# xuekt98/BBDM

Hardware: AMD Instinct MI355X
Metric: denoise-UNet sampling steps/sec (one step = p_sample of the whole local batch: UNet forward + Brownian-Bridge update) at 256x256 pixel-space BBDM (higher is better)
Workload: dtype f32 (tile GEMMs: fp32 operands as two fp16 planes under a provable power-of-two scale, 3 fp16-MFMA terms, fp32 accumulate -- measured against fp64 MORE accurate than the six-term bf16x3 split and than the f32 MFMA; 1x1 layers (skip / qkv / proj_out) and the long-sequence attention: the same pair; sh; 1 GPU; pixel-space BBDM 256x256, batch 16, 1000-step schedule (BASELINE.json configs[1]); batch_per_gpu=16, image_size=256, schedule_steps=1000, parallelism=dp1 (independent image-pair shards)

## Files before the change

bbdm_amd/csrc/common.h:

```cpp
#pragma once
#include <hip/hip_runtime.h>
#include <stdint.h>
#include <stdio.h>
#include "../../include/bbdm_hip.h"

typedef float f32x4 __attribute__((ext_vector_type(4)));
typedef float f32x16 __attribute__((ext_vector_type(16)));

#define BBDM_WAVE 64

void bbdm_set_error(const char* fmt, ...);

enum BbdmOption { BBDM_OPT_WGRAD1X1_BF3 = 0, BBDM_OPT_WINO_IDX64, BBDM_OPT_BF3P_KERNEL, BBDM_OPT_ATTN_BF3, BBDM_OPT_ATTN_PIPE, BBDM_OPT_BF3P_PAD_ROWS, BBDM_OPT_COUNT };
int bbdm_option(int id);

#define BBDM_REQUIRE(cond, ...)            \
    do {                                   \
        if (!(cond)) {                     \
            bbdm_set_error(__VA_ARGS__);   \
            return BBDM_E_BADARG;          \
        }                                  \
    } while (0)

#define BBDM_CHECK_LAUNCH(what)                                                        \
    do {                                                                               \
        hipError_t e__ = hipGetLastError();                                            \
        if (e__ != hipSuccess) {                                                       \
            bbdm_set_error("%s: launch failed: %s", what, hipGetErrorString(e__));     \
            return BBDM_E_LAUNCH;                                                      \
        }                                                                              \
    } while (0)

constexpr int BBDM_MAX_DEVICES = 64;
static inline int bbdm_device_slot() {
    int d = 0;
    if (hipGetDevice(&d) != hipSuccess || d < 0 || d >= BBDM_MAX_DEVICES) d = 0;
    return d;
}
template <auto Kernel>
static inline int bbdm_ensure_lds(size_t bytes, const char* what) {
    static size_t set_dev[BBDM_MAX_DEVICES] = {};
    size_t& set = set_dev[bbdm_device_slot()];
    if (bytes <= set) return BBDM_OK;
    if (hipFuncSetAttribute(reinterpret_cast<const void*>(Kernel), hipFuncAttributeMaxDynamicSharedMemorySize, (int)bytes) != hipSuccess) {
        bbdm_set_error("%s: hipFuncSetAttribute(%zu B LDS) failed", what, bytes);
        return BBDM_E_LAUNCH;
    }
    set = bytes;
    return BBDM_OK;
}

int bbdm_gemm_tn_impl(const float* A, int lda, size_t a_stride, const float* B, int ldb, size_t b_stride, float* C, float* bias_part,
                      int batch, long long K, int M, int N, void* stream);

namespace {
__global__ void bbdm_zero8_kernel(unsigned long long* __restrict__ p, size_t n) {
    for (size_t i = blockIdx.x * (size_t)blockDim.x + threadIdx.x; i < n; i += (size_t)gridDim.x * blockDim.x) p[i] = 0ull;
}
}
static inline void bbdm_zero_async(void* p, size_t bytes, hipStream_t st) {
    const size_t n = bytes / 8;
    if (!n) return;
    size_t blocks = (n + 255) / 256;
    if (blocks > 2048) blocks = 2048;
    hipLaunchKernelGGL(bbdm_zero8_kernel, dim3((unsigned)blocks), dim3(256), 0, st, (unsigned long long*)p, n);
}
// ... 73 lines not shown
```

bbdm_amd/csrc/runtime.hip:

```cpp
#include <stdarg.h>
#include <string.h>
#include "common.h"

static thread_local char g_err[512] = "";

void bbdm_set_error(const char* fmt, ...) {
    va_list ap;
    va_start(ap, fmt);
    vsnprintf(g_err, sizeof(g_err), fmt, ap);
    va_end(ap);
}

extern "C" int bbdm_version(void) { return 33; }

namespace {
struct Option { const char* name; int value; };
Option g_options[BBDM_OPT_COUNT] = {
    {"wgrad1x1_bf3", 1},
    {"wino_idx64", 0},
    {"bf3p_kernel", 6},
    {"attn_bf3", 1},
    {"attn_pipe", 2},
    {"bf3p_pad_rows", 1},
};
int option_index(const char* name) {
    if (!name) return -1;
    for (int i = 0; i < BBDM_OPT_COUNT; ++i)
        if (strcmp(name, g_options[i].name) == 0) return i;
    return -1;
}
}
int bbdm_option(int id) { return g_options[id].value; }
extern "C" int bbdm_set_option(const char* name, int value) {
    const int i = option_index(name);
    BBDM_REQUIRE(i >= 0, "bbdm_set_option: unknown option '%s'", name ? name : "(null)");
    g_options[i].value = value;
    return BBDM_OK;
}
extern "C" int bbdm_get_option(const char* name, int* value) {
    const int i = option_index(name);
    BBDM_REQUIRE(i >= 0 && value, "bbdm_get_option: unknown option '%s' / null result", name ? name : "(null)");
    *value = g_options[i].value;
    return BBDM_OK;
}
extern "C" const char* bbdm_last_error(void) { return g_err; }

namespace {
int device_cus() {
    static int cus_dev[BBDM_MAX_DEVICES] = {};
    int& cus = cus_dev[bbdm_device_slot()];
    if (!cus) {
        int dev = 0;
        hipDeviceProp_t prop;
        cus = (hipGetDevice(&dev) == hipSuccess && hipGetDeviceProperties(&prop, dev) == hipSuccess && prop.multiProcessorCount > 0)
                  ? prop.multiProcessorCount : 256;
    }
    return cus;
}
}

extern "C" int bbdm_device_cus(void) { return device_cus(); }
```

bbdm_amd/csrc/winograd.hip:

```cpp
#include "winograd_math.h"
#include "dispatch.h"
#include <stdlib.h>
#include "bf3_split.h"
#include "h2_split.h"
#include "stats_acc.h"

namespace {

constexpr int KC = 16;

template <int MO, bool PRE, bool UP>
__global__ void __launch_bounds__(256) winograd_input_kernel(const float* __restrict__ x, int ldx, float* __restrict__ V,
                                                             const float* __restrict__ sc, const float* __restrict__ bi,
                                                             int pre_ld, int pre_silu, int N, int H, int W, int C,
                                                             size_t plane) {
    constexpr int AL = MO + 2;
    const int C4 = C >> 2;
    const int TH = H / MO, TW = W / MO;
    const long long total = (long long)N * TH * TW * C4;
    for (long long u = blockIdx.x * 256ll + threadIdx.x; u < total; u += (long long)gridDim.x * 256) {
        const int c = (int)(u % C4) * 4;
        const long long tile = u / C4;
        const int tw = (int)(tile % TW);
        const long long r = tile / TW;
// ... 208 lines not shown
            }
            bt_transform<MO>(d, col);
#pragma unroll
            for (int i = 0; i < AL; ++i) t[i][j] = col[i];
            __builtin_amdgcn_sched_barrier(0);
        }
        float* o = V + (size_t)tile * C + c;
#pragma unroll
        for (int i = 0; i < AL; ++i) {
            float2 row[AL];
            bt_transform<MO>(t[i], row);
#pragma unroll
            for (int j = 0; j < AL; ++j) { *reinterpret_cast<float2*>(o) = row[j]; o += plane; }
            __builtin_amdgcn_sched_barrier(0);
        }
    }
}


template <int AL, int NPL = 3>
__device__ __forceinline__ void store_transposed(const unsigned (&pl)[AL][NPL], unsigned char* scratch, int lane, unsigned char* dst_xi0,
                                                 size_t plane_t, int chunk, int tile0, int tchunks) {
    typedef short v4s __attribute__((ext_vector_type(4)));
    constexpr int HALF = AL / 2, COMBOS = NPL * HALF, PITCH = 256 + 64;
    static_assert(COMBOS * PITCH <= AL * 64 * 8, "transposition scratch exceeds the wave's LDS region");
    const int grp = lane >> 4, i16 = lane & 15;
    const int c = chunk * KC + i16;
    unsigned char* dst = dst_xi0 + (((size_t)(c >> 5) * tchunks + (tile0 >> 4)) * NPL) * 1024 + ((tile0 >> 3) & 1) * 512 + (c & 31) * 16;
#pragma unroll
    for (int round = 0; round < 2; ++round) {
        __builtin_amdgcn_wave_barrier();
#pragma unroll
        for (int q = 0; q < HALF; ++q)
#pragma unroll
            for (int p = 0; p < NPL; ++p)
                *reinterpret_cast<unsigned*>(scratch + (q * NPL + p) * PITCH + lane * 4) = pl[round * HALF + q][p];
        __builtin_amdgcn_wave_barrier();
#pragma unroll
        for (int it = 0; it < (COMBOS + 3) / 4; ++it) {
            const int combo = it * 4 + grp;
            const int cc = combo < COMBOS ? combo : COMBOS - 1;
            const unsigned char* a = scratch + cc * PITCH + (i16 >> 2) * 32 + (i16 & 3) * 8;
            const v4s lo = __builtin_amdgcn_ds_read_tr16_b64_v4i16((__attribute__((address_space(3))) v4s*)(a));
            const v4s hi = __builtin_amdgcn_ds_read_tr16_b64_v4i16((__attribute__((address_space(3))) v4s*)(a + 4 * 32));
            typedef short v8s __attribute__((ext_vector_type(8)));
            const v8s both = {lo[0], lo[1], lo[2], lo[3], hi[0], hi[1], hi[2], hi[3]};
            const int q = cc / NPL, p = cc - NPL * q;
            if (combo < COMBOS)
                *reinterpret_cast<uint4*>(dst + (size_t)(round * HALF + q) * plane_t + p * 1024) = __builtin_bit_cast(uint4, both);
        }
    }
}

struct GnFold {
    const unsigned long long* stats;
    const float* gamma;
    const float* beta;
    const float* film;
    int film_ld, C, G, cpg;
    double cnt;
    float eps;
};
template <int MO, bool PRE, bool UP, bool TR, bool IDX64, bool GNC = false, bool F32 = false, int ST = MO, int NPL = 3>
__global__ void __launch_bounds__((MO + 2) * 64) winograd_input_split2_kernel(const float* __restrict__ x, int ldx,
                                                                              unsigned char* __restrict__ Vp,
                                                                              const float* __restrict__ sc, const float* __restrict__ bi,
                                                                              int pre_ld, int pre_silu, int N, int H, int W, int nchunks,
                                                                              unsigned T, int TG, size_t plane,
                                                                              unsigned char* __restrict__ Vt, size_t plane_t,
                                                                              int tchunks, const FastDiv dTW, const FastDiv dTH,
                                                                              const FastDiv dCH, const GnFold gn,
                                                                              const float* __restrict__ hbound, int vt_h2 = 0) {
    static_assert(NPL == 3 || (NPL == 2 && !F32), "the fp16-pair planes have no fp32 form");
    constexpr int AL = MO + 2;
    __shared__ float2 lds[AL * AL * 64];
    const unsigned L = blockIdx.x, q = L >> 3;
    const unsigned qc = fastdiv(q, dCH);
    const int chunk = (int)(q - qc * (unsigned)nchunks), tg = (int)(qc * 8 + (L & 7));
    if (tg >= TG) return;
    const int lane = threadIdx.x & 63, wave = threadIdx.x >> 6;
    const int TH = (int)dTH.d, TW = (int)dTW.d;
    constexpr int TPG = F32 ? 4 : 8, CPW = F32 ? 16 : 8;
    const int tl = lane / CPW, cp = lane % CPW;
    const unsigned tile = (unsigned)tg * TPG + tl;
    const int c = chunk * (2 * CPW) + cp * 2;
    {
        const int jj = wave;
        float2 d[AL], col[AL];
        if (tile < T) {
            const unsigned r = fastdiv(tile, dTW), n = fastdiv(r, dTH);
            const int tw = (int)(tile - r * (unsigned)TW), th = (int)(r - n * (unsigned)TH);
            float2 s2 = make_float2(1.f, 1.f), b2 = make_float2(0.f, 0.f);
            if (PRE && GNC) {
                const unsigned long long* cell = gn.stats + (((size_t)n * gn.G + c / gn.cpg) * 2) * SA_W;
                const double s = sa_load(cell), ss = sa_load(cell + SA_W);
                const double mean = s / gn.cnt;
                double var = ss / gn.cnt - mean * mean;
                var = var > 0.0 ? var : 0.0;
                const float rstd = (float)(1.0 / sqrt(var + (double)gn.eps));
                const float fmean = (float)mean;
                const float2 ga = *reinterpret_cast<const float2*>(gn.gamma + c), be = *reinterpret_cast<const float2*>(gn.beta + c);
                float sc0 = rstd * ga.x, sc1 = rstd * ga.y;
                float bi0 = be.x - fmean * sc0, bi1 = be.y - fmean * sc1;
                if (gn.film) {
                    const float2 fs = *reinterpret_cast<const float2*>(gn.film + (size_t)n * gn.film_ld + c);
                    const float2 fb = *reinterpret_cast<const float2*>(gn.film + (size_t)n * gn.film_ld + gn.C + c);
                    sc0 = sc0 * (1.f + fs.x); sc1 = sc1 * (1.f + fs.y);
                    bi0 = bi0 * (1.f + fs.x) + fb.x; bi1 = bi1 * (1.f + fs.y) + fb.y;
                }
                s2 = make_float2(sc0, sc1);
                b2 = make_float2(bi0, bi1);
            } else if (PRE) {
                s2 = *reinterpret_cast<const float2*>(sc + (size_t)n * pre_ld + c);
                b2 = *reinterpret_cast<const float2*>(bi + (size_t)n * pre_ld + c);
            }
            const int Hs = UP ? H >> 1 : H, Ws = UP ? W >> 1 : W;
            const int w = ST * tw - 1 + jj;
            const int wc = min(max(w, 0), W - 1);
            const int wsrc = UP ? wc >> 1 : wc;
            const float wmask = (w >= 0 && w < W) ? 1.f : 0.f;
            const int h0 = ST * th - 1;
            if (IDX64) {
#pragma unroll
                for (int i = 0; i < AL; ++i) {
                    const int hc = min(max(h0 + i, 0), H - 1);
                    const int hs = UP ? hc >> 1 : hc;
                    d[i] = *reinterpret_cast<const float2*>(x + ((size_t)(n * Hs + hs) * Ws + wsrc) * ldx + c);
                }
            } else {
                const unsigned rowstride = (unsigned)Ws * (unsigned)ldx;
                const unsigned e0 = (n * (unsigned)Hs * (unsigned)Ws + (unsigned)wsrc) * (unsigned)ldx + (unsigned)c;
// ... 206 lines not shown
#pragma unroll
#if BBDM_NT_MLOAD
            for (int i = 0; i < AL; ++i) v[i] = load_nt(reinterpret_cast<const float2*>(m + (size_t)(i * AL + j) * plane));
#else
            for (int i = 0; i < AL; ++i) v[i] = *reinterpret_cast<const float2*>(m + (size_t)(i * AL + j) * plane);
#endif
            at_transform<MO>(v, sj);
#pragma unroll
            for (int a = 0; a < MO; ++a) s[a][j] = sj[a];
        }
        const float2 b2 = bias ? *reinterpret_cast<const float2*>(bias + c) : make_float2(0.f, 0.f);
        double psum = 0.0, psq = 0.0;
#pragma unroll
        for (int a = 0; a < MO; ++a) {
            float2 o[MO];
            at_transform<MO>(s[a], o);
            const int oh = MO * th + a;
            const int ohc = min(oh, H - 1);
            float2 rv[MO];
            if (RES) {
#pragma unroll
                for (int b = 0; b < MO; ++b) {
                    const int owc = min(MO * tw + b, W - 1);
                    const float* rp = res_per_image == 1 ? res + (size_t)n * ldr + c
                                      : res_per_image == 2 ? res + ((size_t)(n * (H >> 1) + (ohc >> 1)) * (W >> 1) + (owc >> 1)) * ldr + c
                                                           : res + ((size_t)(n * H + ohc) * W + owc) * ldr + c;
                    rv[b] = *reinterpret_cast<const float2*>(rp);
                }
            }
#pragma unroll
            for (int b = 0; b < MO; ++b) {
                const int ow = MO * tw + b;
                if (oh < H && ow < W) {
                    float2 val = o[b] + b2;
                    if (RES) val = val + rv[b];
                    const size_t pix = ph ? (size_t)(n * 2 * H + 2 * oh + (pq >> 1)) * (2 * W) + 2 * ow + (pq & 1)
                                          : (size_t)(n * H + oh) * W + ow;
                    *reinterpret_cast<float2*>(y + pix * ldy + c) = val;
                    if (stats) {
                        psum += (double)val.x + (double)val.y;
                        psq += (double)val.x * val.x + (double)val.y * val.y;
                    }
                }
            }
        }
        if (stats) stat_add(lsum, st, n - n0, n, c, psum, psq);
    }
    if (stats) {
        __syncthreads();
        stat_flush(lsum, st, n0, N);
    }
}

template <int MO, bool RES, int TPW, int AL = MO + 2>
__global__ void __launch_bounds__(AL * 64) winograd_output_lds_kernel(const float* __restrict__ M, size_t plane, int ldm, int splits,
                                                                   const float* __restrict__ bias,
                                                                   const float* __restrict__ res, int ldr, int res_per_image,
                                                                   float* __restrict__ y, int ldy, int N, int H, int W, int Cout,
                                                                   int cblocks, long long T, const StatArgs st, int ph, int tpw) {
    constexpr int NT = AL * 64, NBUF = TPW > 1 ? 2 : 1;
    constexpr int GL = 33;
    constexpr int TAB = MO * 2 * 2 * GL * 2;
    constexpr int XF = NBUF * MO * AL * 64;
    constexpr bool DYN = (size_t)XF * sizeof(float2) > 65536;
    __shared__ float2 lds_static[DYN ? 1 : (XF > TAB ? XF : TAB)];
    extern __shared__ __attribute__((aligned(16))) float2 lds_dynamic[];
    float2* const lds = DYN ? lds_dynamic : lds_static;
    const int lane = threadIdx.x & 63, wave = threadIdx.x >> 6;
    const int cb = (int)(blockIdx.x % (unsigned)cblocks);
    const long long tile0 = (long long)(blockIdx.x / (unsigned)cblocks) * tpw;
    const int TH = wino_tdim(H, MO), TW = wino_tdim(W, MO);
    const int n0 = (int)(tile0 / ((long long)TH * TW));
    const int cm = cb * 128 + 2 * lane;
    const int pq = ph ? cm / Cout : 0, c = cm - pq * Cout;
    const bool stats = st.s[0] != nullptr || st.s[1] != nullptr;
    double acc_s[2] = {0.0, 0.0}, acc_q[2] = {0.0, 0.0};
    const float2 b2 = bias ? *reinterpret_cast<const float2*>(bias + c) : make_float2(0.f, 0.f);
    for (int k = 0; k < tpw; ++k) {
        const long long tile = tile0 + k;
        if (tile >= T) break;
        float2* buf = lds + (k & (NBUF - 1)) * (MO * AL * 64);
        {
            const int j = wave;
            const float* m = M + (size_t)tile * ldm + cm + (size_t)j * plane;
            float2 v[AL], sj[MO];
#pragma unroll
            for (int i = 0; i < AL; ++i) v[i] = load_nt(reinterpret_cast<const float2*>(m + (size_t)(i * AL) * plane));
            for (int z = 1; z < splits; ++z)
#pragma unroll
                for (int i = 0; i < AL; ++i)
                    v[i] = v[i] + load_nt(reinterpret_cast<const float2*>(m + ((size_t)z * (AL * AL) + i * AL) * plane));
            if constexpr (MO == 7) at_transform7(v, sj); else at_transform<MO>(v, sj);
#pragma unroll
            for (int a = 0; a < MO; ++a) buf[(a * AL + j) * 64 + lane] = sj[a];
        }
        __syncthreads();
        if (wave < MO) {
            const int a = wave;
            const int tw = (int)(tile % TW);
            const long long r = tile / TW;
            const int th = (int)(r % TH), n = (int)(r / TH);
            float2 t[AL], o[MO];
#pragma unroll
            for (int j = 0; j < AL; ++j) t[j] = buf[(a * AL + j) * 64 + lane];
            const int oh = MO == 7 ? MO * th + a - (pq >> 1) : MO * th + a;
            if (oh < H && (MO != 7 || oh >= 0)) {
                float2 rv[MO];
                if (RES) {
#pragma unroll
                    for (int b = 0; b < MO; ++b) {
                        const int owc = min(MO * tw + b, W - 1);
                        const float* rp = res_per_image == 1 ? res + (size_t)n * ldr + c
                                          : res_per_image == 2 ? res + ((size_t)(n * (H >> 1) + (oh >> 1)) * (W >> 1) + (owc >> 1)) * ldr + c
                                                               : res + ((size_t)(n * H + oh) * W + owc) * ldr + c;
                        rv[b] = *reinterpret_cast<const float2*>(rp);
                    }
                }
                if constexpr (MO == 7) at_transform7(t, o); else at_transform<MO>(t, o);
                double psum = 0.0, psq = 0.0;
#pragma unroll
                for (int b = 0; b < MO; ++b) {
                    const int ow = MO == 7 ? MO * tw + b - (pq & 1) : MO * tw + b;
                    if (ow < W && (MO != 7 || ow >= 0)) {
                        float2 val = o[b] + b2;
                        if (RES) val = val + rv[b];
                        const size_t pix = ph ? (size_t)(n * 2 * H + 2 * oh + (pq >> 1)) * (2 * W) + 2 * ow + (pq & 1)
                                              : (size_t)(n * H + oh) * W + ow;
                        *reinterpret_cast<float2*>(y + pix * ldy + c) = val;
                        if (stats) {
                            psum += (double)val.x + (double)val.y;
                            psq += (double)val.x * val.x + (double)val.y * val.y;
                        }
                    }
                }
                if (stats) {
                    if (n == n0) { acc_s[0] += psum; acc_q[0] += psq; } else { acc_s[1] += psum; acc_q[1] += psq; }
                }
            }
        }
        if (NBUF == 1 && tpw > 1) __syncthreads();
    }
    if (stats) {
        double* tab = reinterpret_cast<double*>(lds);
        static_assert(sizeof(double) == sizeof(float2), "the table is parked in the float2 transform buffer");
        const int c_first = c - 2 * lane;
        __syncthreads();
        if (wave < MO) {
#pragma unroll
            for (int k = 0; k < 2; ++k) {
                if (!st.s[k]) continue;
                const int g = (st.coff[k] + c) / st.cpg[k], g_first = (st.coff[k] + c_first) / st.cpg[k];
                const bool tail = sa_seg_tail(g, lane);
#pragma unroll
                for (int sl = 0; sl < 2; ++sl) {
                    double vs = acc_s[sl], vq = acc_q[sl];
                    sa_seg_scan2(vs, vq, g, lane, st.cpg[k] >> 1);
                    if (tail) {
                        double* t = tab + ((((size_t)wave * 2 + k) * 2 + sl) * GL + (g - g_first)) * 2;
                        t[0] = vs; t[1] = vq;
                    }
                }
            }
        }
        __syncthreads();
        for (int i = threadIdx.x; i < 2 * 2 * GL * 2; i += NT) {
            const int which = i & 1, gl = (i >> 1) % GL, sl = ((i >> 1) / GL) & 1, k = (i >> 1) / (2 * GL);
            if (!st.s[k]) continue;
            const int n = n0 + sl;
            const int g_first = (st.coff[k] + c_first) / st.cpg[k], g_last = (st.coff[k] + c_first + 127) / st.cpg[k];
            const int g = g_first + gl;
// ... 284 lines not shown
extern "C" int bbdm_winograd_gemm_f32(int m, const float* V, const float* packed_wino, float* M, int N, int H, int W,
                                      int CinPad, int Cout, void* stream) {
    BBDM_WINO_M8(m);
    BBDM_REQUIRE(V && packed_wino && M && N > 0, "winograd_gemm: null pointer / bad N");
    BBDM_WINO_HW(m, H, W);
    BBDM_REQUIRE(CinPad > 0 && CinPad % 4 == 0 && Cout % 4 == 0 && Cout > 0, "winograd_gemm: bad channel counts");
    BBDM_REQUIRE((((uintptr_t)V | (uintptr_t)M | (uintptr_t)packed_wino) & 15) == 0, "winograd_gemm: 16-byte alignment");
    const size_t Tp = tiles_padded(N, H, W, m);
    BBDM_REQUIRE(Tp * (size_t)CinPad < (1ull << 32), "winograd_gemm: one transformed plane exceeds 2^32 elements");
    const size_t wz = bbdm_winograd_packed_floats(m, Cout, CinPad) / planes(m);
    return bbdm_conv1x1_batched(V, CinPad, Tp * (size_t)CinPad, packed_wino, wz, M, Cout, Tp * (size_t)Cout, planes(m),
                                (int)(Tp / 32), 32, CinPad, Cout, (hipStream_t)stream);
}

extern "C" int bbdm_winograd_gemm_bf3_f32(int m, const float* V, const void* packed_bf3, float* M, int N, int H, int W,
                                          int CinPad, int Cout, void* stream) {
    BBDM_WINO_M8(m);
    BBDM_REQUIRE(V && packed_bf3 && M && N > 0, "winograd_gemm_bf3: null pointer / bad N");
    BBDM_WINO_HW(m, H, W);
    return bbdm_gemm_bf3_f32(V, packed_bf3, M, planes(m), (long long)tiles_padded(N, H, W, m), CinPad, Cout, stream);
}

static int winograd_input_planes(int m, const float* x, int ldx, void* Vp, void* Vt, const float* pre_scale, const float* pre_bias,
                                 int pre_ld, int pre_silu, int upsample, int N, int H, int W, int CinPad, void* stream,
                                 const GnFold* fold, bool f32out, const float* hbound, int vt_h2) {
    BBDM_WINO_M78(m);
    BBDM_REQUIRE(!hbound || !f32out, "winograd_input_h2p: the fp16-pair planes have no fp32 form");
    BBDM_REQUIRE(m != 7 || (!upsample && !Vt && !fold && !f32out), "winograd_input_bf3p: m = 7 (phase filters) takes x itself, planes only");
    BBDM_REQUIRE(m != 8 || !fold, "winograd_input_bf3p: m = 8 is a tile of the large layers (no coefficient folding)");
    BBDM_REQUIRE(x && Vp && N > 0, "winograd_input_bf3p: null pointer / bad N");
    BBDM_WINO_HW(m, H, W);
    BBDM_REQUIRE(!upsample || (H % 2 == 0 && W % 2 == 0), "winograd_input_bf3p: upsample needs even H, W");
    BBDM_REQUIRE(CinPad > 0 && CinPad % KC == 0 && ldx % 2 == 0 && ldx >= CinPad, "winograd_input_bf3p: CinPad=%d ldx=%d", CinPad, ldx);
    BBDM_REQUIRE(((uintptr_t)x & 7) == 0 && ((uintptr_t)Vp & 15) == 0, "winograd_input_bf3p: alignment");
    BBDM_REQUIRE((pre_scale == nullptr) == (pre_bias == nullptr), "winograd_input_bf3p: pre_scale / pre_bias must come together");
    BBDM_REQUIRE(!pre_scale || (pre_ld % 2 == 0 && pre_ld >= CinPad && (((uintptr_t)pre_scale | (uintptr_t)pre_bias) & 7) == 0),
                 "winograd_input_bf3p: pre_ld / alignment of the fused-producer coefficients");
    const size_t T = tiles_raw(N, H, W, m), Tp = tiles_padded(N, H, W, m);
    int nchunks = CinPad / KC, TG = (int)(Tp / 8);
    const size_t plane = Tp * (size_t)CinPad * (f32out || hbound ? 4 : 6);
    const size_t plane_t = (size_t)((CinPad + 31) / 32 * 32) * Tp * (vt_h2 ? 4 : 6);
    BBDM_REQUIRE(!Vt || (!upsample && ((uintptr_t)Vt & 15) == 0), "winograd_input_bf3p: the transposed copy needs upsample = 0, 16-B alignment");
    hipStream_t st = (hipStream_t)stream;
    const long long blocks = 8ll * ((TG + 7) / 8) * nchunks;
    BBDM_REQUIRE(blocks < (1ll << 31) && Tp < (1ull << 31), "winograd_input_bf3p: too many workgroups / tiles");
    dim3 g((unsigned)blocks);
    const int Hs = upsample ? H / 2 : H, Ws = upsample ? W / 2 : W;
    const int idx64_env = bbdm_option(BBDM_OPT_WINO_IDX64);
    const bool idx64 = idx64_env || (unsigned long long)N * Hs * Ws * (unsigned long long)ldx >= (1ull << 32) ||
                       (unsigned long long)Ws * (unsigned long long)ldx >= (1ull << 24) || Hs >= (1 << 24);
    const FastDiv dTW = fastdiv_make((unsigned)wino_tdim(W, m)), dTH = fastdiv_make((unsigned)wino_tdim(H, m));
    FastDiv dCH = fastdiv_make((unsigned)nchunks);
    const GnFold gn = fold ? *fold : GnFold{};
    const char* what = "winograd_input_bf3p";
    auto launch = [&](auto MO, auto PRE, auto UP, auto TR, auto I64, auto GNC, auto F32, auto ST, auto NPL) {
        hipLaunchKernelGGL((winograd_input_split2_kernel<MO(), PRE(), UP(), TR(), I64(), GNC(), F32(), ST(), NPL()>), g, dim3((MO() + 2) * 64),
                           0, st, x, ldx, (unsigned char*)Vp, GNC() ? nullptr : pre_scale, GNC() ? nullptr : pre_bias, pre_ld, pre_silu, N, H, W,
                           nchunks, (unsigned)T, TG, plane, TR() ? (unsigned char*)Vt : nullptr, plane_t, (int)(Tp / 16), dTW, dTH, dCH, gn,
                           hbound, vt_h2);
        BBDM_CHECK_LAUNCH(what);
        return BBDM_OK;
    };
    const auto pre = pre_scale != nullptr, up = upsample != 0;
    const auto npl = one_of<3, 2>(hbound ? 2 : 3);
    if (m == 7) {
        what = "winograd_input_bf3p(m = 7)";
        return dispatch([&](auto PRE, auto I64, auto NPL) { return launch(int_c<6>, PRE, no_tag, no_tag, I64, no_tag, no_tag, int_c<7>, NPL); },
                        pre, idx64, npl);
    }
    if (fold) {
        BBDM_REQUIRE(!idx64 && !Vt, "winograd_input_bf3p_gn: tensor too large for the coefficient-folding variant");
        what = "winograd_input_bf3p_gn";
        return dispatch([&](auto MO, auto UP, auto NPL) { return launch(MO, yes_tag, UP, no_tag, no_tag, yes_tag, no_tag, MO, NPL); },
                        one_of<2, 4, 6>(m), up, npl);
    }
    if (f32out) {
        BBDM_REQUIRE(!Vt && CinPad % 32 == 0, "winograd_input: the fp32 form has no transposed copy and takes whole 32-channel chunks");
        nchunks = CinPad / 32, TG = (int)(Tp / 4);
        dCH = fastdiv_make((unsigned)nchunks);
        g = dim3((unsigned)(8ll * ((TG + 7) / 8) * nchunks));
        BBDM_REQUIRE(8ll * ((TG + 7) / 8) * nchunks < (1ll << 31), "winograd_input: too many workgroups");
        what = "winograd_input(fp32 rows, two-phase)";
        return dispatch([&](auto MO, auto PRE, auto UP, auto I64) { return launch(MO, PRE, UP, no_tag, I64, no_tag, yes_tag, MO, int_c<3>); },
                        one_of<2, 4, 8, 6>(m), pre, up, idx64);
    }
    if (Vt)
        return dispatch([&](auto MO, auto PRE, auto I64, auto NPL) { return launch(MO, PRE, no_tag, yes_tag, I64, no_tag, no_tag, MO, NPL); },
                        one_of<2, 4, 8, 6>(m), pre, idx64, npl);
    return dispatch([&](auto MO, auto PRE, auto UP, auto I64, auto NPL) { return launch(MO, PRE, UP, no_tag, I64, no_tag, no_tag, MO, NPL); },
                    one_of<2, 4, 8, 6>(m), pre, up, idx64, npl);
}

extern "C" int bbdm_winograd_input_bf3p_f32(int m, const float* x, int ldx, void* Vp, const float* pre_scale,
                                            const float* pre_bias, int pre_ld, int pre_silu, int upsample, int N, int H, int W,
                                            int CinPad, void* stream) {
    return winograd_input_planes(m, x, ldx, Vp, nullptr, pre_scale, pre_bias, pre_ld, pre_silu, upsample, N, H, W, CinPad, stream, nullptr, false);
}

static int winograd_input_planes_gn(const char* name, bool h2, int m, const float* x, int ldx, void* Vp, const void* stats, int C, int pre_silu,
                                    int upsample, int N, int H, int W, int CinPad, const float* gamma, const float* beta, const float* film,
                                    int film_ld, int HW, int G, float eps, const float* vbound, void* stream) {
    BBDM_REQUIRE(stats && gamma && beta && (!h2 || vbound), "%s: null pointer", name);
    BBDM_REQUIRE(C == CinPad && G > 0 && C % G == 0 && (C / G) % 2 == 0 && HW > 0 && (!film || film_ld >= 2 * C),
                 "%s: C=%d CinPad=%d G=%d HW=%d film_ld=%d", name, C, CinPad, G, HW, film_ld);
    BBDM_REQUIRE((((uintptr_t)gamma | (uintptr_t)beta | (uintptr_t)film) & 7) == 0 && (!film || film_ld % 2 == 0),
                 "%s: gamma / beta / film must be 8-byte aligned", name);
    GnFold f;
    f.stats = (const unsigned long long*)stats; f.gamma = gamma; f.beta = beta; f.film = film;
    f.film_ld = film_ld; f.C = C; f.G = G; f.cpg = C / G; f.cnt = (double)HW * (double)(C / G); f.eps = eps;
    return winograd_input_planes(m, x, ldx, Vp, nullptr, nullptr, nullptr, C, pre_silu, upsample, N, H, W, CinPad, stream, &f, false, vbound);
}
extern "C" int bbdm_winograd_input_bf3p_gn_f32(int m, const float* x, int ldx, void* Vp, const void* stats, const void* unused, int C,
// ... 73 lines not shown
}

extern "C" int bbdm_winograd_output_splitk_stats_f32(int m, const float* M, const float* bias, const float* residual, int ldr,
                                                     float* out, int ldo, int flags, int N, int H, int W, int Cout, void* stats0,
                                                     int cpg0, int coff0, void* stats1, int cpg1, int coff1, int splits,
                                                     void* stream) {
    BBDM_WINO_M78(m);
    BBDM_REQUIRE(splits >= 1 && (splits == 1 || m < 6), "winograd_output: splits=%d (m = 6 / 7 / 8 layers are never split)", splits);
    BBDM_REQUIRE(m != 7 || ((flags & BBDM_CONV_OUT_PHASES) && Cout % 128 == 0),
                 "winograd_output: m = 7 is the phase-filter form (BBDM_CONV_OUT_PHASES, Cout %% 128 == 0)");
    BBDM_REQUIRE(M && out && N > 0, "winograd_output: null pointer / bad N");
    BBDM_WINO_HW(m, H, W);
    BBDM_REQUIRE(Cout > 0 && Cout % 4 == 0 && ldo % 4 == 0 && ldo >= Cout, "winograd_output: Cout=%d ldo=%d", Cout, ldo);
    BBDM_REQUIRE((flags & ~(BBDM_CONV_RES_PER_IMAGE | BBDM_CONV_RES_UPSAMPLE | BBDM_CONV_OUT_PHASES)) == 0 &&
                     (flags & (BBDM_CONV_RES_PER_IMAGE | BBDM_CONV_RES_UPSAMPLE)) != (BBDM_CONV_RES_PER_IMAGE | BBDM_CONV_RES_UPSAMPLE),
                 "winograd_output: unsupported flags 0x%x", flags);
    const int ph = (flags & BBDM_CONV_OUT_PHASES) ? 1 : 0;
    BBDM_REQUIRE(!ph || (!residual && splits == 1), "winograd_output: BBDM_CONV_OUT_PHASES takes neither a residual nor split-K partials");
    const int Cm = ph ? 4 * Cout : Cout;
    BBDM_REQUIRE(!(flags & BBDM_CONV_RES_UPSAMPLE) || (residual && H % 2 == 0 && W % 2 == 0),
                 "winograd_output: BBDM_CONV_RES_UPSAMPLE needs a residual and even H, W");
    BBDM_REQUIRE(!residual || (ldr % 4 == 0 && ldr >= Cout && ((uintptr_t)residual & 15) == 0), "winograd_output: ldr=%d", ldr);
    BBDM_REQUIRE(!bias || ((uintptr_t)bias & 15) == 0, "winograd_output: bias alignment");
    BBDM_REQUIRE((((uintptr_t)M | (uintptr_t)out) & 15) == 0, "winograd_output: 16-byte alignment");
    BBDM_REQUIRE((!stats0 || (cpg0 > 0 && cpg0 % 4 == 0 && coff0 >= 0 && (coff0 + Cout - 1) / cpg0 < 32)) &&
                     (!stats1 || (cpg1 > 0 && cpg1 % 4 == 0 && coff1 >= 0 && (coff1 + Cout - 1) / cpg1 < 32)),
                 "winograd_output: statistics targets need cpg %% 4 == 0 and (coff + Cout) / cpg <= 32");
    StatArgs st;
    st.s[0] = (unsigned long long*)stats0; st.cpg[0] = cpg0 > 0 ? cpg0 : 1; st.coff[0] = coff0;
    st.s[1] = (unsigned long long*)stats1; st.cpg[1] = cpg1 > 0 ? cpg1 : 1; st.coff[1] = coff1;
    const size_t T = tiles_raw(N, H, W, m), Tp = tiles_padded(N, H, W, m);
    const long long units = (long long)T * (Cm / (m == 6 ? 2 : 4));
    long long iters = units / (256ll * 6144);
    iters = iters < 1 ? 1 : (iters > 16 ? 16 : iters);
    const long long blocks = (units + 256 * iters - 1) / (256 * iters);
    BBDM_REQUIRE(blocks < (1ll << 31), "winograd_output: too many workgroups");
    const int rpi = (flags & BBDM_CONV_RES_PER_IMAGE) ? 1 : (flags & BBDM_CONV_RES_UPSAMPLE) ? 2 : 0;
    const dim3 g((unsigned)blocks), b(256);
    hipStream_t s_ = (hipStream_t)stream;
    if (Cm % 128 == 0 && (!ph || Cout % 128 == 0) && (long long)T * (Cm / 128) < (1ll << 31)) {
        int tpw = 2;
        if (stats0 || stats1) {
            int cells = 0;
            if (stats0) cells += 2 * (128 / st.cpg[0] + 1);
            if (stats1) cells += 2 * (128 / st.cpg[1] + 1);
            tpw = cells / 8;
            if (tpw < 2) tpw = 2;
            if (tpw > 8) tpw = 8;
            while (tpw > 2 && ((long long)((T + tpw - 1) / tpw) * (Cm / 128) < 2048)) --tpw;
        }
        const long long per_image = (long long)wino_tdim(H, m) * wino_tdim(W, m);
        if (tpw > per_image) tpw = (int)per_image;
        if (tpw < 1) tpw = 1;
        auto launch = [&](auto MO, auto RES, auto TPW, auto AL, size_t lds, const char* what) {
            hipLaunchKernelGGL((winograd_output_lds_kernel<MO(), RES(), TPW(), AL()>), dim3((unsigned)(((T + tpw - 1) / tpw) * (size_t)(Cm / 128))),
                               dim3(AL() * 64), lds, s_, M, Tp * (size_t)Cm, Cm, splits, bias, residual, ldr, rpi, out, ldo, N, H, W, Cout,
                               Cm / 128, (long long)T, st, ph, tpw);
            BBDM_CHECK_LAUNCH(what);
            return BBDM_OK;
        };
        const auto one_tile = one_of<1, 2>(tpw == 1 ? 1 : 2);
        if (m == 7)
            return dispatch([&](auto TPW) { return launch(int_c<7>, no_tag, TPW, int_c<8>, 0, "winograd_output(m = 7)"); }, one_tile);
        if (m == 8) {
            constexpr size_t lds8 = (size_t)2 * 8 * 10 * 64 * sizeof(float2);
            if (tpw < 2) tpw = per_image >= 2 ? 2 : 1;
            return dispatch([&](auto RES) {
                if (const int rc = bbdm_ensure_lds<winograd_output_lds_kernel<8, RES(), 2>>(lds8, "winograd_output")) return rc;
                return launch(int_c<8>, RES, int_c<2>, int_c<10>, lds8, "winograd_output");
            }, residual != nullptr);
        }
        return dispatch([&](auto MO, auto TPW, auto RES) { return launch(MO, RES, TPW, int_c<MO() + 2>, 0, "winograd_output"); },
                        one_of<6, 4, 2>(m), one_tile, residual != nullptr);
    }
    BBDM_REQUIRE(m != 7 && m != 8, "winograd_output: m = 7 / 8 need Cout %% 128 == 0 (the two-phase kernel)");
    if (m == 6)
        return dispatch([&](auto RES) {
            hipLaunchKernelGGL(winograd_output6_kernel<RES()>, g, b, 0, s_, M, Tp * (size_t)Cm, Cm, bias, residual, ldr, rpi, out,
                               ldo, N, H, W, Cout, (int)iters, st, ph);
            BBDM_CHECK_LAUNCH("winograd_output");
            return BBDM_OK;
        }, residual != nullptr);
    return dispatch([&](auto MO) {
        hipLaunchKernelGGL(winograd_output_kernel<MO()>, g, b, 0, s_, M, Tp * (size_t)Cm, Cm, splits, bias, residual, ldr, rpi, out,
                           ldo, N, H, W, Cout, (int)iters, st, ph);
        BBDM_CHECK_LAUNCH("winograd_output");
        return BBDM_OK;
    }, one_of<2, 4>(m));
}

extern "C" int bbdm_winograd_output_stats_f32(int m, const float* M, const float* bias, const float* residual, int ldr,
                                              float* out, int ldo, int flags, int N, int H, int W, int Cout, void* stats0,
                                              int cpg0, int coff0, void* stats1, int cpg1, int coff1,
                                              void* stream) {
    return bbdm_winograd_output_splitk_stats_f32(m, M, bias, residual, ldr, out, ldo, flags, N, H, W, Cout, stats0, cpg0, coff0,
                                                 stats1, cpg1, coff1, 1, stream);
}

extern "C" int bbdm_winograd_output_f32(int m, const float* M, const float* bias, const float* residual, int ldr,
                                        float* out, int ldo, int flags, int N, int H, int W, int Cout, void* stream) {
    return bbdm_winograd_output_stats_f32(m, M, bias, residual, ldr, out, ldo, flags, N, H, W, Cout, nullptr, 0, 0, nullptr, 0,
                                          0, stream);
}

extern "C" int bbdm_conv3x3_winograd_f32(int m, const float* x, int ldx, const float* packed_wino, const float* bias,
                                         const float* residual, int ldr, float* out, int ldo, int flags, float* ws, int N,
                                         int H, int W, int CinPad, int Cout, void* stream) {
    BBDM_WINO_M8(m);
    BBDM_REQUIRE(ws, "winograd: null workspace");
    BBDM_REQUIRE(N > 0 && H > 0 && W > 0 && CinPad > 0, "winograd: bad shape");
    float* V = ws;
    float* M = ws + (size_t)planes(m) * tiles_padded(N, H, W, m) * CinPad;
    int rc = bbdm_winograd_input_f32(m, x, ldx, V, nullptr, nullptr, 0, 0, 0, N, H, W, CinPad, stream);
    if (rc == BBDM_OK) rc = bbdm_winograd_gemm_f32(m, V, packed_wino, M, N, H, W, CinPad, Cout, stream);
    if (rc == BBDM_OK) rc = bbdm_winograd_output_f32(m, M, bias, residual, ldr, out, ldo, flags, N, H, W, Cout, stream);
    return rc;
}

static int winograd_dy_planes(int m, const float* dy, int ld, void* dMt, float* dm11, int N, int H, int W, int Cout, const float* dybound,
                              void* stream);
extern "C" int bbdm_winograd_dy_transform_bf3p_f32(int m, const float* dy, int ld, void* dMt, float* dm11, int N, int H, int W,
                                                   int Cout, void* stream) {
    return winograd_dy_planes(m, dy, ld, dMt, dm11, N, H, W, Cout, nullptr, stream);
}
extern "C" int bbdm_winograd_dy_transform_h2p_f32(int m, const float* dy, int ld, void* dMt, float* dm11, int N, int H, int W,
                                                  int Cout, const float* dybound, void* stream) {
// ... 109 lines not shown
```

Baseline: 14.04 steps/s.

## Band-walk Winograd input tiles per XCD and prefetch residuals early in output kernel

Adds a banded workgroup-to-tile mapping for the Winograd input transform (m=8, wide images). Each XCD's workgroups walk a contiguous band of tile rows and a small set of channel chunks, which should improve L2 locality on the chiplet-partitioned cache. The m=8 output kernel with a residual now issues its residual loads before the A-transform and LDS exchange, hiding their latency, and sets a launch-bounds occupancy hint. In exchange it adds extra index arithmetic per block and holds more registers for the residuals across the barrier.

```diff
diff --git a/bbdm_amd/csrc/common.h b/bbdm_amd/csrc/common.h
--- a/bbdm_amd/csrc/common.h
+++ b/bbdm_amd/csrc/common.h
@@ -11,7 +11,7 @@
 
 void bbdm_set_error(const char* fmt, ...);
 
-enum BbdmOption { BBDM_OPT_WGRAD1X1_BF3 = 0, BBDM_OPT_WINO_IDX64, BBDM_OPT_BF3P_KERNEL, BBDM_OPT_ATTN_BF3, BBDM_OPT_ATTN_PIPE, BBDM_OPT_BF3P_PAD_ROWS, BBDM_OPT_COUNT };
+enum BbdmOption { BBDM_OPT_WGRAD1X1_BF3 = 0, BBDM_OPT_WINO_IDX64, BBDM_OPT_BF3P_KERNEL, BBDM_OPT_ATTN_BF3, BBDM_OPT_ATTN_PIPE, BBDM_OPT_BF3P_PAD_ROWS, BBDM_OPT_WINO_XCD_BAND, BBDM_OPT_COUNT };
 int bbdm_option(int id);
 
 #define BBDM_REQUIRE(cond, ...)            \
diff --git a/bbdm_amd/csrc/runtime.hip b/bbdm_amd/csrc/runtime.hip
--- a/bbdm_amd/csrc/runtime.hip
+++ b/bbdm_amd/csrc/runtime.hip
@@ -22,6 +22,7 @@
     {"attn_bf3", 1},
     {"attn_pipe", 2},
     {"bf3p_pad_rows", 1},
+    {"wino_xcd_band", 1},
 };
 int option_index(const char* name) {
     if (!name) return -1;
diff --git a/bbdm_amd/csrc/winograd.hip b/bbdm_amd/csrc/winograd.hip
--- a/bbdm_amd/csrc/winograd.hip
+++ b/bbdm_amd/csrc/winograd.hip
@@ -284,6 +284,25 @@
     }
 }
 
+struct BandWalk {
+    unsigned B, S, nsub, nsets;
+    FastDiv dSub;
+    FastDiv dSet, dSetL;
+    FastDiv dC, dCL;
+};
+constexpr int WINO_BAND_ROWS = 16, WINO_BAND_LINES = 4;
+constexpr int WINO_BAND_MIN_TW = 16;
+static inline BandWalk band_walk_make(unsigned B, unsigned nchunks, unsigned S, unsigned CS) {
+    BandWalk w;
+    S = S < 1 ? 1 : (S > B ? B : S);
+    CS = CS < 1 ? 1 : (CS > nchunks ? nchunks : CS);
+    w.B = B; w.S = S; w.nsub = (B + S - 1) / S; w.nsets = (nchunks + CS - 1) / CS;
+    const unsigned Sl = B - (w.nsub - 1) * S, CSl = nchunks - (w.nsets - 1) * CS;
+    w.dSub = fastdiv_make(S * nchunks);
+    w.dSet = fastdiv_make(S * CS); w.dSetL = fastdiv_make(Sl * CS);
+    w.dC = fastdiv_make(CS); w.dCL = fastdiv_make(CSl);
+    return w;
+}
 struct GnFold {
     const unsigned long long* stats;
     const float* gamma;
@@ -302,13 +321,27 @@
                                                                               unsigned char* __restrict__ Vt, size_t plane_t,
                                                                               int tchunks, const FastDiv dTW, const FastDiv dTH,
                                                                               const FastDiv dCH, const GnFold gn,
-                                                                              const float* __restrict__ hbound, int vt_h2 = 0) {
+                                                                              const float* __restrict__ hbound, int vt_h2,
+                                                                              const BandWalk bw) {
     static_assert(NPL == 3 || (NPL == 2 && !F32), "the fp16-pair planes have no fp32 form");
     constexpr int AL = MO + 2;
     __shared__ float2 lds[AL * AL * 64];
     const unsigned L = blockIdx.x, q = L >> 3;
-    const unsigned qc = fastdiv(q, dCH);
-    const int chunk = (int)(q - qc * (unsigned)nchunks), tg = (int)(qc * 8 + (L & 7));
+    int chunk, tg;
+    if (bw.B) {
+        const unsigned sb = fastdiv(q, bw.dSub);
+        unsigned r = q - sb * bw.dSub.d;
+        const bool lsb = sb + 1 == bw.nsub;
+        const unsigned cs = fastdiv(r, lsb ? bw.dSetL : bw.dSet);
+        r -= cs * (lsb ? bw.dSetL.d : bw.dSet.d);
+        const bool lcs = cs + 1 == bw.nsets;
+        const unsigned gi = fastdiv(r, lcs ? bw.dCL : bw.dC);
+        chunk = (int)(cs * bw.dC.d + (r - gi * (lcs ? bw.dCL.d : bw.dC.d)));
+        tg = (int)((L & 7) * bw.B + sb * bw.S + gi);
+    } else {
+        const unsigned qc = fastdiv(q, dCH);
+        chunk = (int)(q - qc * (unsigned)nchunks), tg = (int)(qc * 8 + (L & 7));
+    }
     if (tg >= TG) return;
     const int lane = threadIdx.x & 63, wave = threadIdx.x >> 6;
     const int TH = (int)dTH.d, TW = (int)dTW.d;
@@ -621,8 +654,9 @@
     }
 }
 
-template <int MO, bool RES, int TPW, int AL = MO + 2>
-__global__ void __launch_bounds__(AL * 64) winograd_output_lds_kernel(const float* __restrict__ M, size_t plane, int ldm, int splits,
+constexpr int wino_out_waves(int MO, bool EARLY) { return EARLY && MO == 8 ? 5 : 0; }
+template <int MO, bool RES, int TPW, int AL = MO + 2, bool EARLY = false>
+__global__ void __launch_bounds__(AL * 64, wino_out_waves(MO, EARLY)) winograd_output_lds_kernel(const float* __restrict__ M, size_t plane, int ldm, int splits,
                                                                    const float* __restrict__ bias,
                                                                    const float* __restrict__ res, int ldr, int res_per_image,
                                                                    float* __restrict__ y, int ldy, int N, int H, int W, int Cout,
@@ -649,6 +683,25 @@
         const long long tile = tile0 + k;
         if (tile >= T) break;
         float2* buf = lds + (k & (NBUF - 1)) * (MO * AL * 64);
+        int tw = 0, th = 0, n = 0, oh = 0;
+        float2 rv[MO];
+        auto locate = [&]() {
+            tw = (int)(tile % TW);
+            const long long r = tile / TW;
+            th = (int)(r % TH), n = (int)(r / TH);
+            oh = MO == 7 ? MO * th + wave - (pq >> 1) : MO * th + wave;
+        };
+        auto row_in_image = [&]() { return oh < H && (MO != 7 || oh >= 0); };
+        auto fetch_residuals = [&]() {
+#pragma unroll
+            for (int b = 0; b < MO; ++b) {
+                const int owc = min(MO * tw + b, W - 1);
+                const float* rp = res_per_image == 1 ? res + (size_t)n * ldr + c
+                                  : res_per_image == 2 ? res + ((size_t)(n * (H >> 1) + (oh >> 1)) * (W >> 1) + (owc >> 1)) * ldr + c
+                                                       : res + ((size_t)(n * H + oh) * W + owc) * ldr + c;
+                rv[b] = *reinterpret_cast<const float2*>(rp);
+            }
+        };
         {
             const int j = wave;
             const float* m = M + (size_t)tile * ldm + cm + (size_t)j * plane;
@@ -659,6 +712,29 @@
 #pragma unroll
                 for (int i = 0; i < AL; ++i)
                     v[i] = v[i] + load_nt(reinterpret_cast<const float2*>(m + ((size_t)z * (AL * AL) + i * AL) * plane));
+            bool own = false;
+            const float* rrow = res;
+            int rsh = 0, rstep = 0;
+            if constexpr (RES && EARLY) {
+                if (wave < MO) {
+                    locate();
+                    own = row_in_image();
+                }
+                if (own) {
+                    rrow = res_per_image == 1 ? res + (size_t)n * ldr + c
+                           : res_per_image == 2 ? res + ((size_t)(n * (H >> 1) + (oh >> 1)) * (W >> 1)) * ldr + c
+                                                : res + ((size_t)(n * H + oh) * W) * ldr + c;
+                    rsh = res_per_image == 2 ? 1 : 0;
+                    rstep = res_per_image == 1 ? 0 : ldr;
+                }
+            }
+            if constexpr (RES && EARLY) {
+                if (own) {
+#pragma unroll
+                    for (int b = 0; b < MO; ++b)
+                        rv[b] = *reinterpret_cast<const float2*>(rrow + (size_t)(min(MO * tw + b, W - 1) >> rsh) * rstep);
+                }
+            }
             if constexpr (MO == 7) at_transform7(v, sj); else at_transform<MO>(v, sj);
 #pragma unroll
             for (int a = 0; a < MO; ++a) buf[(a * AL + j) * 64 + lane] = sj[a];
@@ -666,25 +742,12 @@
         __syncthreads();
         if (wave < MO) {
             const int a = wave;
-            const int tw = (int)(tile % TW);
-            const long long r = tile / TW;
-            const int th = (int)(r % TH), n = (int)(r / TH);
+            if constexpr (!(RES && EARLY)) locate();
             float2 t[AL], o[MO];
 #pragma unroll
             for (int j = 0; j < AL; ++j) t[j] = buf[(a * AL + j) * 64 + lane];
-            const int oh = MO == 7 ? MO * th + a - (pq >> 1) : MO * th + a;
-            if (oh < H && (MO != 7 || oh >= 0)) {
-                float2 rv[MO];
-                if (RES) {
-#pragma unroll
-                    for (int b = 0; b < MO; ++b) {
-                        const int owc = min(MO * tw + b, W - 1);
-                        const float* rp = res_per_image == 1 ? res + (size_t)n * ldr + c
-                                          : res_per_image == 2 ? res + ((size_t)(n * (H >> 1) + (oh >> 1)) * (W >> 1) + (owc >> 1)) * ldr + c
-                                                               : res + ((size_t)(n * H + oh) * W + owc) * ldr + c;
-                        rv[b] = *reinterpret_cast<const float2*>(rp);
-                    }
-                }
+            if (row_in_image()) {
+                if constexpr (RES && !EARLY) fetch_residuals();
                 if constexpr (MO == 7) at_transform7(t, o); else at_transform<MO>(t, o);
                 double psum = 0.0, psq = 0.0;
 #pragma unroll
@@ -1075,12 +1138,20 @@
     const FastDiv dTW = fastdiv_make((unsigned)wino_tdim(W, m)), dTH = fastdiv_make((unsigned)wino_tdim(H, m));
     FastDiv dCH = fastdiv_make((unsigned)nchunks);
     const GnFold gn = fold ? *fold : GnFold{};
+    const int band_opt = bbdm_option(BBDM_OPT_WINO_XCD_BAND);
+    const int band_rows = band_opt > 255 ? (band_opt >> 8 > 65535 ? 65535 : band_opt >> 8) : WINO_BAND_ROWS, band_lines = band_opt > 255 ? band_opt & 255 : WINO_BAND_LINES;
+    auto walk = [&]() {
+        if (!band_opt || (band_opt <= 255 && (m != 8 || wino_tdim(W, m) < WINO_BAND_MIN_TW))) return BandWalk{};
+        const unsigned tpg = f32out ? 4 : 8, lines = f32out ? 1 : 2;
+        const unsigned row_groups = ((unsigned)wino_tdim(W, m) + tpg - 1) / tpg;
+        return band_walk_make((unsigned)((TG + 7) / 8), (unsigned)nchunks, (unsigned)band_rows * row_groups, (unsigned)band_lines * lines);
+    };
     const char* what = "winograd_input_bf3p";
     auto launch = [&](auto MO, auto PRE, auto UP, auto TR, auto I64, auto GNC, auto F32, auto ST, auto NPL) {
         hipLaunchKernelGGL((winograd_input_split2_kernel<MO(), PRE(), UP(), TR(), I64(), GNC(), F32(), ST(), NPL()>), g, dim3((MO() + 2) * 64),
                            0, st, x, ldx, (unsigned char*)Vp, GNC() ? nullptr : pre_scale, GNC() ? nullptr : pre_bias, pre_ld, pre_silu, N, H, W,
                            nchunks, (unsigned)T, TG, plane, TR() ? (unsigned char*)Vt : nullptr, plane_t, (int)(Tp / 16), dTW, dTH, dCH, gn,
-                           hbound, vt_h2);
+                           hbound, vt_h2, walk());
         BBDM_CHECK_LAUNCH(what);
         return BBDM_OK;
     };
@@ -1260,26 +1331,30 @@
         const long long per_image = (long long)wino_tdim(H, m) * wino_tdim(W, m);
         if (tpw > per_image) tpw = (int)per_image;
         if (tpw < 1) tpw = 1;
-        auto launch = [&](auto MO, auto RES, auto TPW, auto AL, size_t lds, const char* what) {
-            hipLaunchKernelGGL((winograd_output_lds_kernel<MO(), RES(), TPW(), AL()>), dim3((unsigned)(((T + tpw - 1) / tpw) * (size_t)(Cm / 128))),
+        auto launch = [&](auto MO, auto RF, auto TPW, auto AL, size_t lds, const char* what) {
+            hipLaunchKernelGGL((winograd_output_lds_kernel<MO(), RF() != 0, TPW(), AL(), RF() == 2>),
+                               dim3((unsigned)(((T + tpw - 1) / tpw) * (size_t)(Cm / 128))),
                                dim3(AL() * 64), lds, s_, M, Tp * (size_t)Cm, Cm, splits, bias, residual, ldr, rpi, out, ldo, N, H, W, Cout,
                                Cm / 128, (long long)T, st, ph, tpw);
             BBDM_CHECK_LAUNCH(what);
             return BBDM_OK;
         };
         const auto one_tile = one_of<1, 2>(tpw == 1 ? 1 : 2);
+        const auto res_form = one_of<0, 1, 2>(!residual ? 0 : (m == 8 && bbdm_option(BBDM_OPT_WINO_XCD_BAND)) ? 2 : 1);
         if (m == 7)
-            return dispatch([&](auto TPW) { return launch(int_c<7>, no_tag, TPW, int_c<8>, 0, "winograd_output(m = 7)"); }, one_tile);
+            return dispatch([&](auto TPW) { return launch(int_c<7>, int_c<0>, TPW, int_c<8>, 0, "winograd_output(m = 7)"); }, one_tile);
         if (m == 8) {
             constexpr size_t lds8 = (size_t)2 * 8 * 10 * 64 * sizeof(float2);
             if (tpw < 2) tpw = per_image >= 2 ? 2 : 1;
-            return dispatch([&](auto RES) {
-                if (const int rc = bbdm_ensure_lds<winograd_output_lds_kernel<8, RES(), 2>>(lds8, "winograd_output")) return rc;
-                return launch(int_c<8>, RES, int_c<2>, int_c<10>, lds8, "winograd_output");
-            }, residual != nullptr);
-        }
-        return dispatch([&](auto MO, auto TPW, auto RES) { return launch(MO, RES, TPW, int_c<MO() + 2>, 0, "winograd_output"); },
-                        one_of<6, 4, 2>(m), one_tile, residual != nullptr);
+            return dispatch([&](auto RF) {
+                if (const int rc = bbdm_ensure_lds<winograd_output_lds_kernel<8, RF() != 0, 2, 10, RF() == 2>>(lds8, "winograd_output")) return rc;
+                return launch(int_c<8>, RF, int_c<2>, int_c<10>, lds8, "winograd_output");
+            }, res_form);
+        }
+        return dispatch([&](auto MO, auto TPW, auto RF) {
+            if constexpr (RF() == 2) return (int)BBDM_E_BADARG;
+            else return launch(MO, RF, TPW, int_c<MO() + 2>, 0, "winograd_output");
+        }, one_of<6, 4, 2>(m), one_tile, res_form);
     }
     BBDM_REQUIRE(m != 7 && m != 8, "winograd_output: m = 7 / 8 need Cout %% 128 == 0 (the two-phase kernel)");
     if (m == 6)
```

Result: no change. 14.09 steps/s (median of 6 runs) (+0.4%).
